# aleph-zero-foundation/sha2-on-cq-halo2

Measured on AMD Instinct MI355X. Metric: sha256_cq_create_proof_k18: MSM Mscalar/s over proof-generation wall-clock (ms_per_step), higher is better.
Workload: dtype u256-montgomery

## Files before the change

### sha2_on_cq_halo2_amd/csrc/capi_msm.hip

```cpp
#include <algorithm>
#include <cstdlib>
#include <cstring>
#include <string>
#include <vector>
#include "ctx.hpp"
#include "msm.hpp"
#include "g1fft.hpp"
#include "setup.hpp"
#include "cq.hpp"
#include "serde.hpp"
#include "msm_g2.hpp"

using namespace cq;

uint32_t msm_table_window_bits(size_t n) {
  if (const char* e = getenv("CQ_TABLE_C")) {
    const long v = atol(e);
    if (v >= (long)MSM_TABLE_C_MIN && v <= (long)MSM_TABLE_C_MAX) return (uint32_t)v;
  }
  return n >= ((size_t)1 << 20) ? 17u : MSM_TABLE_C;
}

static uint32_t pick_c(cq_ctx* c, uint32_t n) {
  if (c->msm_c) return c->msm_c;
// ... 243 lines not shown
  c->msm_precompute = on != 0;
  return CQ_OK;
}

int cq_msm_set_table_window(cq_ctx* c, uint32_t bits) {
  if (!c || (bits != 0 && (bits < MSM_TABLE_C_MIN || bits > MSM_TABLE_C_MAX))) return CQ_ERR_ARG;
  c->msm_table_c = bits;
  return CQ_OK;
}

int cq_msm_table_width_dev(cq_ctx* c, const uint64_t* bases_dev, size_t n, uint32_t preferred_bits, uint32_t* bits) {
  if (!c || !bases_dev || !bits) return CQ_ERR_ARG;
  const cq_ctx::MsmTable* t = c->find_msm_table(bases_dev, n, nullptr, preferred_bits);
  *bits = t ? t->c : 0;
  return CQ_OK;
}

int cq_msm_bucket_sums_dev(cq_ctx* c, const uint64_t* const* bases_dev, size_t arrays, int packed, const uint32_t* index_dev, size_t n,
                           size_t buckets, uint64_t* out_dev) {
  if (!c || !bases_dev || !index_dev || !out_dev || !arrays || arrays > MSM_MAX_BATCH || !n || n > ((size_t)1 << 26) || !buckets ||
      buckets > ((size_t)1 << (MSM_TABLE_C - 1)))
    return CQ_ERR_ARG;
  CQ_HIP(c, hipSetDevice(c->device));
  void *sc, *conv = nullptr;
  int rc;
  if ((rc = c->ensure_scratch(Scratch::EntryA, n * sizeof(Fr), &sc)) != CQ_OK) return rc;
  if (!packed && (rc = c->ensure_scratch(Scratch::EntryB, arrays * n * sizeof(G1Affine), &conv)) != CQ_OK) return rc;
  if (msm_index_scalars(c, index_dev, (uint32_t)n, (uint32_t)buckets, (Fr*)sc) != 0) return c->fail(CQ_ERR_HIP, "bucket sums: scalars");
  std::vector<const Fr*> scal(arrays, (const Fr*)sc);
  std::vector<const G1Affine*> bs(arrays);
  for (size_t a = 0; a < arrays; a++) {
    if (!bases_dev[a]) return CQ_ERR_ARG;
    bs[a] = (const G1Affine*)bases_dev[a];
    if (!packed) {
      G1Affine* dst = (G1Affine*)conv + a * n;
      if (msm_bases29(c, bs[a], (uint32_t)n, dst) != 0) return c->fail(CQ_ERR_HIP, "bucket sums: bases");
      bs[a] = dst;
    }
  }
  if (msm_bucket_sums(c, scal.data(), bs.data(), (uint32_t)n, (uint32_t)arrays, (uint32_t)buckets, (G1Affine*)out_dev) != 0)
    return c->fail(CQ_ERR_HIP, "bucket-sum launch failed");
  return c->wait(c->stream);
}

int cq_msm_set_window(cq_ctx* c, uint32_t bits) {
  if (!c || (bits != 0 && (bits < 2 || bits > 15))) return CQ_ERR_ARG;
  c->msm_c = bits;
  return CQ_OK;
}

int cq_best_multiexp_dev(cq_ctx* c, const uint64_t* coeffs_dev, const uint64_t* bases_dev, size_t len,
                         uint64_t out_jac[12]) {
  if (!c || !out_jac || (len && (!coeffs_dev || !bases_dev))) return CQ_ERR_ARG;
  CQ_HIP(c, hipSetDevice(c->device));
  const Fr* sc = (const Fr*)coeffs_dev;
  return msm_batch(c, &sc, (const G1Affine*)bases_dev, len, 1, out_jac);
}

int cq_msm_batch_dev(cq_ctx* c, const uint64_t* const* coeffs_dev, const uint64_t* bases_dev, size_t len,
                     size_t count, uint64_t* out_jac) {
  if (!c || !out_jac || !coeffs_dev || (len && !bases_dev)) return CQ_ERR_ARG;
  CQ_HIP(c, hipSetDevice(c->device));
  return msm_batch(c, (const Fr* const*)coeffs_dev, (const G1Affine*)bases_dev, len, count, out_jac);
// ... 414 lines not shown
```

### sha2_on_cq_halo2_amd/csrc/cq.hip

```cpp
#include "cq.hpp"
#include "ctx.hpp"
#include "tablehash.hpp"

namespace cq {

__global__ void table_insert_kernel(const Fr* __restrict__ values, uint32_t N, uint32_t* __restrict__ slots, uint32_t nslots,
                                    uint32_t* __restrict__ err) {
  const uint32_t i = blockIdx.x * blockDim.x + threadIdx.x;
  if (i >= N) return;
  const Fr v = ld(values + i);
  uint32_t s = hash_fr(v) & (nslots - 1);
  for (uint32_t probe = 0; probe < nslots; probe++) {
    const uint32_t prev = atomicCAS(&slots[s], EMPTY, i);
    if (prev == EMPTY) return;
    if (prev != i && ld(values + prev) == v) {
      atomicExch(err, 1u);
      return;
    }
    s = (s + 1) & (nslots - 1);
  }
  atomicExch(err, 2u);
}

constexpr uint32_t R1_ROWS = 4;
__global__ __launch_bounds__(256) void cq_round1_kernel(CqRound1Batch batch, uint32_t u, uint32_t* __restrict__ err) {
  const CqRound1Args& a = batch.a[blockIdx.y];
  uint32_t* __restrict__ m_counts = batch.m_counts[blockIdx.y];
  Fr* __restrict__ bucket = batch.bucket[blockIdx.y];
  uint32_t found[R1_ROWS];
#pragma unroll
  for (uint32_t r = 0; r < R1_ROWS; r++) {
    const uint32_t row = (blockIdx.x * R1_ROWS + r) * blockDim.x + threadIdx.x;
    uint32_t idx = EMPTY;
    bool bad = row >= u;
    for (uint32_t j = 0; !bad && j < a.width; j++) {
      const Fr v = ld(a.cols[j] + row);
      const uint32_t ix = table_find(a.values[j], a.slots[j], a.nslots[j], v);
      if (ix == EMPTY) {
        atomicExch(err, 1u);
        bad = true;
      } else if (j && ix != idx) {
        atomicExch(err, 2u);
        bad = true;
      }
      idx = ix;
    }
    found[r] = bad ? EMPTY : idx;
    if (bucket && row < batch.n) st(bucket + row, row >= u ? Fr::from_u64(batch.blind_bucket + 1) : bad ? Fr::zero() : Fr::from_u64(idx + 1));
  }
  uint32_t held = EMPTY, held_cnt = 0;
#pragma unroll
  for (uint32_t r = 0; r < R1_ROWS; r++) {
    if (found[r] == EMPTY) continue;
    if (found[r] == held) {
      held_cnt++;
    } else {
      if (held_cnt) atomicAdd(&m_counts[held], held_cnt);
      held = found[r];
      held_cnt = 1;
    }
  }
  bool pending = held_cnt != 0;
#pragma unroll 1
  for (int round = 0; round < 4 && __ballot(pending); round++) {
    const unsigned long long pend = __ballot(pending);
    const int leader = __ffsll((long long)pend) - 1;
    const uint32_t lidx = __shfl(held, leader, 64);
    const bool mine = pending && held == lidx;
    uint32_t c = mine ? held_cnt : 0u;
#pragma unroll
    for (int d = 32; d >= 1; d >>= 1) c += __shfl_xor(c, d, 64);
// ... 304 lines not shown
```

### sha2_on_cq_halo2_amd/csrc/cq.hpp

```cpp
#pragma once
#include <hip/hip_runtime.h>
#include <vector>
#include "../../include/cq_halo2.h"
#include "curve.hpp"
#include "poly.hpp"

struct cq_ctx;
struct cq_params;

namespace cq {

constexpr uint32_t CQ_MAX_WIDTH = 8;

struct CqRound1Args {
  const Fr* cols[CQ_MAX_WIDTH];
  const Fr* values[CQ_MAX_WIDTH];
  const uint32_t* slots[CQ_MAX_WIDTH];
  uint32_t nslots[CQ_MAX_WIDTH];
  uint32_t width;
};
constexpr uint32_t CQ_ROUND1_BATCH = 8;
struct CqRound1Batch {
  CqRound1Args a[CQ_ROUND1_BATCH];
  uint32_t* m_counts[CQ_ROUND1_BATCH];
  Fr* bucket[CQ_ROUND1_BATCH] = {};
  uint32_t blind_bucket = 0, n = 0;
  uint32_t count;
};
struct CqThetaPowers {
  Fr pow[CQ_MAX_WIDTH];
  uint32_t width;
};
constexpr uint32_t CQ_FOLD_BATCH = 8;
struct CqFoldBatch {
  const Fr* src[CQ_FOLD_BATCH][CQ_MAX_WIDTH];
  uint32_t width[CQ_FOLD_BATCH];
  Fr* out[CQ_FOLD_BATCH];
  const Fr* f[CQ_FOLD_BATCH];
  Fr* b[CQ_FOLD_BATCH];
  const uint32_t* m[CQ_FOLD_BATCH];
  Fr* den[CQ_FOLD_BATCH];
  Fr theta_pow[CQ_MAX_WIDTH];
  uint32_t count;
};
int cq_fold_inputs(cq_ctx* c, const CqFoldBatch& b, uint32_t n);
int cq_round2_prep(cq_ctx* c, const CqFoldBatch& b, uint32_t n, uint32_t N, uint32_t u, const Fr& beta);
struct CqAValuesBatch {
  const Fr* den_inv[CQ_FOLD_BATCH];
// ... 141 lines not shown
```

### sha2_on_cq_halo2_amd/csrc/msm.hip

```cpp
#include <algorithm>
#include <cstdlib>
#include "msm.hpp"
#include "curve29.hpp"
#include "ctx.hpp"

namespace cq {

__global__ __launch_bounds__(256) void msm_set_ptrs_kernel(MsmPtrs sc, MsmPtrs bs, MsmStrides st, MsmStrides ln, MsmStrides src, const void** dst,
                                                          uint32_t batch, uint4* __restrict__ zero, size_t zero_quads) {
  CQ_CRITICAL_WAVES();
  for (size_t i = (size_t)blockIdx.x * blockDim.x + threadIdx.x; i < zero_quads; i += (size_t)gridDim.x * blockDim.x)
    zero[i] = make_uint4(0, 0, 0, 0);
  if (blockIdx.x) return;
  const uint32_t t = threadIdx.x;
  if (t < batch) {
    dst[t] = sc.p[t];
    dst[batch + t] = bs.p[t];
    ((uint64_t*)(dst + 2 * batch))[t] = st.s[t];
    ((uint64_t*)(dst + 3 * batch))[t] = ln.s[t];
    ((uint64_t*)(dst + 4 * batch))[t] = src.s[t];
  }
}

static __device__ __forceinline__ uint32_t signed_digit(const U256& v, uint32_t w, uint32_t c, uint32_t& carry, uint32_t& neg) {
// ... 358 lines not shown
__global__ __launch_bounds__(PART_THREADS) void msm_bucket_place_kernel(const uint32_t* __restrict__ part_pay, const uint8_t* __restrict__ part_low,
                                                                        const uint32_t* __restrict__ poff,
                                                                        const uint32_t* __restrict__ off0, uint32_t* __restrict__ cursor,
                                                                        uint32_t* __restrict__ sorted) {
  CQ_CRITICAL_WAVES();
  part_tile_place(BucketBins<PB>{sorted}, part_pay, part_low, poff, off0, cursor);
}
__global__ __launch_bounds__(PART_THREADS) void msm_refine_count_kernel(const uint16_t* __restrict__ low1, const uint32_t* __restrict__ poff1,
                                                                        uint32_t bins_log, uint32_t* __restrict__ psize2) {
  part_count(RefineBins(bins_log), low1, poff1, psize2);
}
__global__ __launch_bounds__(PART_THREADS) void msm_refine_place_kernel(const uint32_t* __restrict__ pay1, const uint16_t* __restrict__ low1,
                                                                        const uint32_t* __restrict__ poff1, uint32_t bins_log,
                                                                        const uint32_t* __restrict__ poff2, uint32_t* __restrict__ cursor2,
                                                                        uint32_t* __restrict__ pay2, uint8_t* __restrict__ low2) {
  part_tile_place(RefineBins(bins_log, pay2, low2), pay1, low1, poff1, poff2, cursor2);
}

__global__ __launch_bounds__(256) void msm_alias_counts_kernel(uint32_t* __restrict__ counts, const uint64_t* __restrict__ list_src, uint32_t B) {
  CQ_CRITICAL_WAVES();
  const uint32_t m = blockIdx.y, src = (uint32_t)list_src[m];
  const uint32_t i = blockIdx.x * blockDim.x + threadIdx.x;
  if (src != m && i < B) counts[(size_t)m * B + i] = counts[(size_t)src * B + i];
}

static __device__ __forceinline__ uint32_t level_value(uint32_t cnt, uint32_t lv, uint32_t s1) {
  if (lv == 0) return cnt;
  uint32_t t = (cnt + s1 - 1) / s1;
  for (uint32_t k = 2; k <= lv; k++) t = t <= MSM_SHORT_MIN ? 0 : (t + MSM_S2 - 1) / MSM_S2;
  return t;
}
static __device__ __forceinline__ uint32_t combine_short_limit(uint32_t slots) {
  return slots <= MSM_WAVE_BUDGET ? MSM_SHORT_MIN : MSM_SHORT;
}

static __device__ __forceinline__ uint32_t block_excl_scan256(uint32_t v, uint32_t* sh , uint32_t& total) {
  const uint32_t lane = threadIdx.x & 63, wid = threadIdx.x >> 6;
  uint32_t x = v;
#pragma unroll
  for (int off = 1; off < 64; off <<= 1) {
    uint32_t y = __shfl_up(x, off, 64);
    if ((int)lane >= off) x += y;
  }
  __syncthreads();
  if (lane == 63) sh[wid] = x;
  __syncthreads();
// ... 240 lines not shown
    r.x = a.x * (iv * a.zzz);
    r.y = a.y * (iv * a.zz);
  }
  store_affine29(next + i, {Fq29::from_mont256(r.x), Fq29::from_mont256(r.y)});
}

int msm_precompute_tables(cq_ctx* ctx, const G1Affine* bases, uint32_t n, uint32_t c, G1Affine* table ) {
  const uint32_t W = (255 + c - 1) / c;
  hipStream_t s = ctx->stream;
  msm_table0_kernel<<<(n + 255) / 256, 256, 0, s>>>(bases, table, n);
  for (uint32_t w = 1; w < W; w++)
    msm_pre_kernel<<<(n + 255) / 256, 256, 0, s>>>(table + (size_t)(w - 1) * n, table + (size_t)w * n, n, c);
  return hipGetLastError() == hipSuccess ? 0 : -1;
}

__global__ __launch_bounds__(256) void msm_bases29_kernel(const G1Affine* bases, G1Affine* out, uint32_t n) {
  const uint32_t i = blockIdx.x * blockDim.x + threadIdx.x;
  if (i >= n) return;
  const Affine29 p = load_affine29(bases + i, true);
  store_affine29(out + i, p);
}
int msm_bases29(cq_ctx* ctx, const G1Affine* bases, uint32_t n, G1Affine* out) {
  msm_bases29_kernel<<<(n + 255) / 256, 256, 0, ctx->stream>>>(bases, out, n);
  return hipGetLastError() == hipSuccess ? 0 : -1;
}
__global__ __launch_bounds__(256) void msm_index_scalars_kernel(const uint32_t* __restrict__ index, uint32_t n, uint32_t count, Fr* __restrict__ out) {
  const uint32_t i = blockIdx.x * blockDim.x + threadIdx.x;
  if (i >= n) return;
  const uint32_t j = index[i];
  out[i] = j < count ? Fr::from_u64(j + 1) : Fr::zero();
}
int msm_index_scalars(cq_ctx* ctx, const uint32_t* index, uint32_t n, uint32_t count, Fr* out) {
  msm_index_scalars_kernel<<<(n + 255) / 256, 256, 0, ctx->stream>>>(index, n, count, out);
  return hipGetLastError() == hipSuccess ? 0 : -1;
}

__global__ __launch_bounds__(256) void msm_buckets_affine_kernel(const XYZZ* __restrict__ buckets, const uint32_t* __restrict__ t1, uint32_t B,
                                                                 uint32_t count, G1Affine* __restrict__ out) {
  const uint32_t i = blockIdx.x * blockDim.x + threadIdx.x, m = blockIdx.y;
  if (i >= count) return;
  const size_t g = (size_t)m * B + i;
  G1Affine r = G1Affine::identity();
  if (t1[g]) {
    const XYZZ29 v = load_xyzz29(buckets + g);
    if (!v.is_identity()) {
      const Fq x = v.x.reduced().to_mont256(), y = v.y.to_mont256(), zz = v.zz.to_mont256(), zzz = v.zzz.to_mont256();
      const Fq iv = (zz * zzz).inv();
      r.x = x * (iv * zzz);
      r.y = y * (iv * zz);
    }
  }
  G1Affine* o = out + (size_t)m * count + i;
  uint32_t w[8];
  for (int k = 0; k < 8; k++) w[k] = r.x.v.l[k];
  st8(&o->x, w);
  for (int k = 0; k < 8; k++) w[k] = r.y.v.l[k];
// ... 354 lines not shown
  off_pairs = o;   o = up(o + (size_t)batch * Wb * (rows + cols) * sizeof(XYZZ));
  total = o;
}

struct PartPass1 {
  hipStream_t s;
  dim3 hgrid, sgrid;
  const Fr* const* scalars;
  const uint64_t *lens, *list_src;
  uint32_t c, W, npart, per_lane, batch, s1, P;
  uint32_t *psize , *poff, *s1_dev, *part_pay;
  void* part_low;
};
template <uint32_t CW, uint32_t NW, typename LowT>
static void launch_part_pass1(const PartPass1& a) {
  msm_part_hist_kernel<CW, NW><<<a.hgrid, DIGITS_LDS_THREADS, 0, a.s>>>(a.scalars, a.lens, a.c, a.W, a.npart, a.per_lane, a.psize);
  msm_part_scan_kernel<<<1, 1024, 0, a.s>>>(a.psize, a.P, a.poff, a.list_src, a.batch, a.npart, a.s1, a.s1_dev);
  msm_part_scatter_kernel<CW, NW, LowT><<<a.sgrid, PSC_THREADS, 0, a.s>>>(a.scalars, a.lens, a.c, a.W, a.npart, a.poff, a.psize + a.P, a.part_pay,
                                                                          (LowT*)a.part_low);
}

int msm_run(cq_ctx* ctx, const Fr* const* scalars_host_ptrs, const G1Affine* const* bases_host_ptrs, const size_t* lens,
            uint32_t n, uint32_t c, uint32_t batch, bool pre, const size_t* table_strides, void* workspace,
            G1Jac* window_sums_dev, G1Affine* raw_out, uint32_t raw_count) {
  hipStream_t s = ctx->stream;
  MsmLayout L(n, c, batch, pre);
  if (pre && (n > (1u << 26) || L.W > 32)) return -4;
  if (L.tmax[0] > 0xfffffff0ull || (uint64_t)batch * L.W * n > 0xfffffff0ull) return -3;
  char* ws = (char*)workspace;
  const Fr** d_scalars = (const Fr**)(ws + L.off_ptrs);
  const G1Affine** d_bases = (const G1Affine**)(ws + L.off_ptrs) + batch;
  uint32_t* ranks = (uint32_t*)(ws + L.off_ranks);
  uint32_t* counts = (uint32_t*)(ws + L.off_counts);
  XYZZ* buckets = (XYZZ*)(ws + L.off_buckets);
  uint32_t* blocksums = (uint32_t*)(ws + L.off_blocksums);
  uint32_t* ticket = (uint32_t*)(ws + L.off_ticket);
  uint32_t* s1_dev = blocksums + (size_t)L.nseq * L.nblk;
  uint32_t* off = (uint32_t*)(ws + L.off_off);
  uint32_t* tk = (uint32_t*)(ws + L.off_tk);
  uint32_t* sorted = (uint32_t*)(ws + L.off_sorted);
  XYZZ* part[2] = {(XYZZ*)(ws + L.off_part[0]), (XYZZ*)(ws + L.off_part[1])};
  XYZZ* pairs = (XYZZ*)(ws + L.off_pairs);
  const uint32_t M = L.M, W = L.W, Bt = L.Bt;
  if (batch == 0 || batch > MSM_MAX_BATCH) return -2;
  MsmPtrs sp, bp;
  MsmStrides stv, lnv, srcv;
  uint32_t alias[MSM_MAX_BATCH];
  bool any_alias = false;
  for (uint32_t i = 0; i < MSM_MAX_BATCH; i++) {
    sp.p[i] = i < batch ? (const void*)scalars_host_ptrs[i] : nullptr;
    bp.p[i] = i < batch ? (const void*)bases_host_ptrs[i] : nullptr;
    stv.s[i] = (i < batch && pre) ? (uint64_t)table_strides[i] : 0;
    lnv.s[i] = i < batch ? (uint64_t)lens[i] : 0;
    alias[i] = i;
    if (i < batch && L.part_sort)
      for (uint32_t j = 0; j < i; j++)
        if (alias[j] == j && scalars_host_ptrs[j] == scalars_host_ptrs[i] && lens[j] == lens[i] && lens[i]) {
          alias[i] = j;
          lnv.s[i] = 0;
          any_alias = true;
          break;
        }
    srcv.s[i] = alias[i];
  }
  const uint64_t* d_strides = (const uint64_t*)((const void**)d_scalars + 2 * batch);
  const uint64_t* d_lens = (const uint64_t*)((const void**)d_scalars + 3 * batch);
  const uint64_t* d_src = (const uint64_t*)((const void**)d_scalars + 4 * batch);
  uint64_t load = 0;
  for (uint32_t i = 0; i < batch; i++) load = std::max<uint64_t>(load, (uint64_t)lens[i] * W / (L.Wb * M));
  const uint32_t partials = pre && L.Wb > 1 ? MSM_PARTIALS_TARGET / 4 : MSM_PARTIALS_TARGET;
  const uint32_t s1 = load <= MSM_S1_BIG_LOAD ? msm_small_launch_s1((uint64_t)batch * W * n)
                                              : std::max<uint32_t>(MSM_S1_BIG, (uint32_t)((load + partials - 1) / partials));
  const uint32_t* off0 = off;
  auto front = [&]() -> int {
  {
    const size_t quads = (L.zero_end - L.off_counts) / sizeof(uint4);
    const uint32_t blocks = (uint32_t)std::min<size_t>((quads + 255) / 256, 1024);
    msm_set_ptrs_kernel<<<std::max(blocks, 1u), 256, 0, s>>>(sp, bp, stv, lnv, srcv, (const void**)d_scalars, batch, (uint4*)counts, quads);
  }
  if (L.part_sort) {
    const uint32_t P = batch * L.npart;
    const uint64_t E = (uint64_t)batch * W * n;
    uint32_t* part_pay = (uint32_t*)(ws + L.off_ranks);
    void* part_low = part_pay + (L.mid ? 2 * E : E);
    uint32_t* poff = (uint32_t*)(ws + L.off_poff);
    uint32_t* cursor = (uint32_t*)(ws + L.off_cursor);
    uint32_t* psize = (uint32_t*)(ws + L.off_psize);
    const uint32_t per_lane = (uint64_t)n * batch <= (1u << 21) ? 2u : DIGITS_LDS_PER_LANE;
    const uint32_t hist_chunk = DIGITS_LDS_THREADS * per_lane;
    const dim3 hgrid((n + hist_chunk - 1) / hist_chunk, batch), sgrid((n + PSC_THREADS - 1) / PSC_THREADS, batch);
    const PartPass1 pp{s, hgrid, sgrid, d_scalars, d_lens, d_src, c, W, L.npart, per_lane, batch, s1, P, psize, poff, s1_dev, part_pay, part_low};
    if (c == 15 && W == 17) launch_part_pass1<15, 17, uint8_t>(pp);
    else if (c == 16 && W == 16) launch_part_pass1<16, 16, uint8_t>(pp);
    else if (c == 17 && W == 15) launch_part_pass1<17, 15, uint8_t>(pp);
    else if (c == 18 && W == 15) launch_part_pass1<18, 15, uint16_t>(pp);
    else if (c == 19 && W == 14) launch_part_pass1<19, 14, uint16_t>(pp);
    else if (c == 20 && W == 13) launch_part_pass1<20, 13, uint16_t>(pp);
    else if (L.mid) launch_part_pass1<0, 0, uint16_t>(pp);
    else launch_part_pass1<0, 0, uint8_t>(pp);
    auto split_for = [&](uint32_t parts) {
      const uint64_t tiles = (uint64_t)W * n * batch / ((uint64_t)parts * PART_TILE) + 1;
      return (uint32_t)std::min<uint64_t>(PART_SPLIT, tiles);
    };
// ... 13 lines not shown
      msm_part_scan_kernel<<<1, 1024, 0, s>>>(psize2, F, poff2);
      msm_refine_place_kernel<<<dim3(P, PART_SPLIT), PART_THREADS, 0, s>>>(part_pay, low1, poff, bins_log, poff2, psize2 + F, pay2, low2);
      fpay = pay2;
      flow = low2;
      fpoff = poff2;
    }
    const uint32_t split = split_for(F);
    const bool wide = !L.mid && L.shift1 == PART_BITS_WIDE;
    if (wide) msm_bucket_count_kernel<PART_BITS_WIDE><<<dim3(F, split), PART_THREADS, 0, s>>>(flow, fpoff, counts);
    else msm_bucket_count_kernel<PART_BITS><<<dim3(F, split), PART_THREADS, 0, s>>>(flow, fpoff, counts);
    if (any_alias) msm_alias_counts_kernel<<<dim3((L.B + 255) / 256, batch), 256, 0, s>>>(counts, d_src, L.B);
    msm_scan_reduce_kernel<<<L.nblk, 256, 0, s>>>(counts, Bt, L.nseq, s1, s1_dev, blocksums, ticket);
    msm_scan_apply_kernel<<<L.nblk, 256, 0, s>>>(counts, Bt, L.nseq, s1, s1_dev, blocksums, off, tk);
    if (wide) msm_bucket_place_kernel<PART_BITS_WIDE><<<dim3(F, split), PART_THREADS, 0, s>>>(fpay, flow, fpoff, off0, cursor, sorted);
    else msm_bucket_place_kernel<PART_BITS><<<dim3(F, split), PART_THREADS, 0, s>>>(fpay, flow, fpoff, off0, cursor, sorted);
  } else {
    msm_digits_kernel<<<dim3((n + 255) / 256, batch), 256, 0, s>>>(d_scalars, d_lens, n, c, W, pre ? 1u : 0u, ranks, counts);
    msm_scan_reduce_kernel<<<L.nblk, 256, 0, s>>>(counts, Bt, L.nseq, s1, nullptr, blocksums, ticket);
    msm_scan_apply_kernel<<<L.nblk, 256, 0, s>>>(counts, Bt, L.nseq, s1, nullptr, blocksums, off, tk);
    msm_scatter_kernel<<<dim3((n + 255) / 256, batch), 256, 0, s>>>(d_scalars, d_lens, n, c, W, pre ? 1u : 0u, ranks, off0, sorted);
  }
  return 0;
  };
  std::vector<uint64_t> sig{(uint64_t)(uintptr_t)workspace, (uint64_t)(uintptr_t)window_sums_dev, n, c, batch, pre ? 1u : 0u, s1,
                            (uint64_t)(uintptr_t)raw_out, raw_count};
  for (uint32_t i = 0; i < batch; i++) {
    sig.push_back((uint64_t)(uintptr_t)scalars_host_ptrs[i]);
    sig.push_back((uint64_t)(uintptr_t)bases_host_ptrs[i]);
    sig.push_back((uint64_t)lens[i]);
    sig.push_back(pre ? (uint64_t)table_strides[i] : 0);
  }
  if (ctx->run_graph(sig, 0, front) != 0) return -1;
  if (ctx->prof_on && ctx->prof_entries && ctx->prof_entries_n < cq_ctx::PROF_COUNTERS)
    (void)hipMemcpyAsync(ctx->prof_entries + ctx->prof_entries_n++, off0 + Bt, sizeof(uint32_t), hipMemcpyDeviceToHost, s);
  constexpr size_t TAIL_EARLY_POINTS = (size_t)1 << 20;
  const bool tail_early = n >= TAIL_EARLY_POINTS;
  if (tail_early && ctx->msm_tail_event) {
    (void)hipEventRecord(ctx->msm_tail_event, s);
    ctx->msm_tail_seq++;
  }
  hipEvent_t pe = ctx->prof_begin(CQ_PROF_MSM_ACCUMULATE);
  msm_accumulate_kernel<<<(uint32_t)((L.tmax[0] + MSM_ACC_THREADS - 1) / MSM_ACC_THREADS), MSM_ACC_THREADS, 0, s>>>(
      d_bases, L.B, pre ? 1u : 0u, d_strides, d_src, sorted, counts, off0, tk, off + (size_t)(Bt + 1), Bt, part[0], buckets);
  ctx->prof_end(pe);
  if (ctx->msm_tail_event && !tail_early) {
    (void)hipEventRecord(ctx->msm_tail_event, s);
    ctx->msm_tail_seq++;
  }
  auto tail = [&]() -> int {
  for (uint32_t k = 1; k < L.levels; k++) {
// ... 19 lines not shown
  const uint32_t sets = batch * L.Wb;
  constexpr uint32_t QUAD_ROWCOL_SETS = 4, SEG32_SETS = 12;
  if (sets <= QUAD_ROWCOL_SETS)
    msm_rowcol_quad_kernel<<<dim3(L.rows + L.cols, sets), 256, 0, s>>>(buckets, tk, M, L.rows, L.cols, pairs);
  else if (sets <= SEG32_SETS)
    msm_rowcol_kernel<32><<<dim3((L.rows + L.cols + 1) / 2, sets), 64, 0, s>>>(buckets, tk, M, L.rows, L.cols, pairs);
  else
    msm_rowcol_kernel<16><<<dim3((L.rows + L.cols + 3) / 4, sets), 64, 0, s>>>(buckets, tk, M, L.rows, L.cols, pairs);
  constexpr uint32_t QUAD_WEIGHTED_WAVES = 2048;
  if (sets * MSM_SET_POINTS * 4 <= QUAD_WEIGHTED_WAVES) msm_weighted_quad_kernel<<<MSM_SET_POINTS * sets, 256, 0, s>>>(pairs, L.rows, L.cols, window_sums_dev);
  else msm_weighted_kernel<<<MSM_SET_POINTS * sets, 64, 0, s>>>(pairs, L.rows, L.cols, window_sums_dev);
  return 0;
  };
  if (ctx->run_graph(sig, 1, tail) != 0) return -1;
  return hipGetLastError() == hipSuccess ? 0 : -1;
}

bool msm_bucket_sums_fit(uint32_t n, uint32_t batch) {
  if (!batch || batch > MSM_MAX_BATCH || !n || n > (1u << 26)) return false;
  MsmLayout L(n, MSM_TABLE_C, batch, true);
  return (uint64_t)batch * L.W * n <= 0xfffffff0ull && L.tmax[0] <= 0xfffffff0ull && L.total <= ((size_t)32 << 30);
}

int msm_bucket_sums(cq_ctx* ctx, const Fr* const* scalars, const G1Affine* const* bases29, uint32_t n, uint32_t batch, uint32_t count,
                    G1Affine* out) {
  const uint32_t c = MSM_TABLE_C;
  if (!count || count > (1u << (c - 1)) || !msm_bucket_sums_fit(n, batch)) return -2;
  MsmLayout L(n, c, batch, true);
  void* ws;
  if (ctx->ensure_scratch(Scratch::MsmWork, L.total, &ws) != 0) return -1;
  const std::vector<size_t> lens(batch, n), strides(batch, n);
  return msm_run(ctx, scalars, bases29, lens.data(), n, c, batch, true, strides.data(), ws, nullptr, out, count);
}

G1Jac msm_set_value(const G1Jac* planes, uint32_t cols) {
  G1Jac v = planes[6];
  for (int t = 5; t >= 0; t--) v = jac_add(jac_dbl(v), planes[t]);
  if (cols == 128) {
    for (int t = 6; t >= 0; t--) v = jac_add(jac_dbl(v), planes[7 + t]);
    return jac_add(v, planes[14]);
  }
  G1Jac u = planes[13];
  for (int t = 5; t >= 0; t--) u = jac_add(jac_dbl(u), planes[7 + t]);
  for (uint32_t l = cols; l > 1; l >>= 1) v = jac_dbl(v);
  return jac_add(jac_add(v, u), planes[14]);
}

G1Jac msm_fold_sets(const G1Jac* pairs, uint32_t Wb, uint32_t M, uint32_t cols) {
  if (Wb == 1) return msm_set_value(pairs, cols);
  G1Jac planes[MSM_SET_POINTS];
  for (uint32_t q = 0; q < MSM_SET_POINTS; q++) {
    planes[q] = pairs[q];
    for (uint32_t s = 1; s < Wb; s++) planes[q] = jac_add(planes[q], pairs[(size_t)MSM_SET_POINTS * s + q]);
  }
  G1Jac acc = msm_set_value(planes, cols);
// ... 29 lines not shown
```

### sha2_on_cq_halo2_amd/csrc/msm.hpp

```cpp
#pragma once
#include <hip/hip_runtime.h>
#include <vector>
#include "curve.hpp"

struct cq_ctx;

namespace cq {

constexpr uint32_t MSM_ACC_THREADS = 128;

#ifndef CQ_MSM_S1
#define CQ_MSM_S1 24
#endif
constexpr uint32_t MSM_S1 = CQ_MSM_S1;
#ifndef CQ_MSM_S1_BIG
#define CQ_MSM_S1_BIG 32
#endif
#ifndef CQ_MSM_S1_BIG_LOAD
#define CQ_MSM_S1_BIG_LOAD 512
#endif
constexpr uint32_t MSM_S1_BIG = CQ_MSM_S1_BIG;
constexpr uint32_t MSM_S1_BIG_LOAD = CQ_MSM_S1_BIG_LOAD;
#ifndef CQ_MSM_PARTIALS_TARGET
#define CQ_MSM_PARTIALS_TARGET 48
// ... 29 lines not shown
#endif
constexpr uint32_t MSM_SHORT_MAX = CQ_MSM_SHORT_MAX;
static_assert(MSM_SHORT_MAX <= MSM_SHORT_LIMIT && MSM_SHORT_MAX >= 4097, "the cut-over covers N + 1 = 4097 and fits the kernel");

struct MsmPtrs {
  const void* p[MSM_MAX_BATCH];
};
struct MsmStrides {
  uint64_t s[MSM_MAX_BATCH];
};

struct MsmLayout {
  uint32_t n, c, batch, W, Wb, M, B, Bt, levels, nseq, nblk, rows, cols, npart, nfinal, shift1;
  bool pre, part_sort, mid;
  uint64_t tmax[8];
  size_t off_ptrs, off_ranks, off_poff, off_poff2, off_counts, off_cursor, off_psize, off_psize2, off_buckets, off_ticket, zero_end, off_blocksums,
      off_off, off_tk, off_sorted, off_part[2], off_pairs, total;
  MsmLayout(uint32_t n_, uint32_t c_, uint32_t batch_, bool pre_ = false);
};

uint32_t msm_window_bits(uint32_t n);
int msm_run(cq_ctx* ctx, const Fr* const* scalars, const G1Affine* const* bases, const size_t* lens, uint32_t n, uint32_t c,
            uint32_t batch, bool pre, const size_t* table_strides, void* workspace, G1Jac* window_sums_dev,
            G1Affine* raw_out = nullptr, uint32_t raw_count = 0);
size_t msm_short_workspace(uint32_t n, uint32_t batch);
int msm_short_run(cq_ctx* ctx, const Fr* const* scalars, const G1Affine* const* bases, uint32_t n, uint32_t batch, void* workspace,
                  G1Jac* window_sums_dev);
int msm_bucket_sums(cq_ctx* ctx, const Fr* const* scalars, const G1Affine* const* bases29, uint32_t n, uint32_t batch, uint32_t count,
                    G1Affine* out);
int msm_bases29(cq_ctx* ctx, const G1Affine* bases, uint32_t n, G1Affine* out);
int msm_index_scalars(cq_ctx* ctx, const uint32_t* index, uint32_t n, uint32_t count, Fr* out);
bool msm_bucket_sums_fit(uint32_t n, uint32_t batch);
int msm_precompute_tables(cq_ctx* ctx, const G1Affine* bases, uint32_t n, uint32_t c, G1Affine* table);
G1Jac msm_set_value(const G1Jac* planes, uint32_t cols);
G1Jac msm_fold_windows(const G1Jac* pairs, uint32_t W, uint32_t c, uint32_t cols);
G1Jac msm_fold_sets(const G1Jac* pairs, uint32_t Wb, uint32_t M, uint32_t cols);

}

int cq_msm_multi(cq_ctx* c, const cq::Fr* const* scalars, const cq::G1Affine* const* bases, size_t len, size_t count,
                 uint64_t* out_jac);
int cq_msm_multi_v(cq_ctx* c, const cq::Fr* const* scalars, const cq::G1Affine* const* bases, const size_t* lens, size_t count,
                   uint64_t* out_jac);
struct MsmPending {
  struct Launch {
    size_t first = 0, slot = 0;
    uint32_t batch = 0, c = 0, nmax = 0, W = 0, Wb = 0, M = 0, cols = 0;
    bool pre = false, empty = false;
    bool short_path = false;
  };
  std::vector<Launch> launches;
  void* host = nullptr;
  size_t slots = 0, count = 0;
};
// ... 10 lines not shown
```

### sha2_on_cq_halo2_amd/csrc/prover.hip

```cpp
#include <algorithm>
#include <array>
#include <atomic>
#include <chrono>
#include <cstdio>
#include <cstdlib>
#include <cstring>
#include <thread>
#include <vector>
#include "blake2b.hpp"
#include "comm.hpp"
#include "cq.hpp"
#include "ctx.hpp"
#include "msm.hpp"
#include "plonk.hpp"
#include "prover.hpp"
#include "glv.hpp"
#include "xoshiro.hpp"

using namespace cq;

namespace {

struct Transcript {
  Blake2b st;
// ... 561 lines not shown
        ga.prog = pk->lookup_prog + lk.prog[j];
        ga.num_polys = 1;
        ga.constants = pk->constants;
        ga.challenges = B.challenges;
        ga.advice = B.adv;
        ga.fixed = pk->fixed_values;
        ga.instance = B.inst_lag;
        ga.stride = n;
        ga.size = (uint32_t)n;
        ga.rot_scale = 1;
        ga.y = Fr::zero();
        Fr* dst = B.lk_inputs + input_slot * n;
        CQ_TRY(gate_eval(c, ga, dst));
        lk_input[l][j] = dst;
      }
      CqRound1Args& ra = r1b.a[r1b.count];
      ra.width = w;
      for (uint32_t j = 0; j < w; j++) {
        ra.cols[j] = lk_input[l][j];
        ra.values[j] = lk.tables[j]->values;
        ra.slots[j] = lk.tables[j]->slots;
        ra.nslots[j] = lk.tables[j]->nslots;
      }
      r1b.bucket[r1b.count] = b_by_rows ? bpoly + l * n : nullptr;
      r1b.n = b_by_rows ? (uint32_t)n : 0;
      r1b.blind_bucket = (uint32_t)N;
      r1b.m_counts[r1b.count++] = m_counts_ + l * N;
      if (r1b.count == CQ_ROUND1_BATCH || l + 1 == L) {
        CQ_TRY(cq_round1(c, r1b, u, err_dev_));
        r1b.count = 0;
      }
    }
    CQ_TRY(cq_m_to_fr(c, m_counts_, (uint32_t)(L * N), B.m_fr));
    for (size_t l0 = 0; b_by_rows && l0 < L; l0 += MSM_MAX_BATCH / 2) {
      std::vector<const Fr*> sc;
      std::vector<const G1Affine*> bs;
      for (size_t l = l0; l < std::min(L, l0 + MSM_MAX_BATCH / 2); l++)
        for (int q = 0; q < 2; q++) { sc.push_back(bpoly + l * n); bs.push_back(pk->b_row_bases[q]); }
      if (msm_bucket_sums(c, sc.data(), bs.data(), (uint32_t)n, (uint32_t)sc.size(), (uint32_t)(N + 1), B.b_sums + 2 * l0 * (N + 1)) != 0)
        return c->fail(CQ_ERR_HIP, "bucket-sum launch failed");
    }
    *herr = 0;
    CQ_HIP(c, hipMemcpyAsync((void*)herr, err_dev_, 4, hipMemcpyDeviceToHost, s));
    return CQ_OK;
  };
  auto lookup_error = [&]() -> int {
    if (*herr == 1) return c->fail(CQ_ERR_LOOKUP, "witness value not in table");
    if (*herr == 2) return c->fail(CQ_ERR_LOOKUP, "Vector lookup must be on the same table row");
    return CQ_OK;
  };
  const bool early_m = L > 0 && pk->num_phases == 1 && pk->challenge_phase.empty();
  std::vector<G1Affine> m_commitments(L, G1Affine::identity());

  const size_t NC = pk->challenge_phase.size();
  std::vector<Fr> user_challenges(NC, Fr::zero());
  std::vector<G1Affine> advice_commitments(A, G1Affine::identity());
  auto phase_of = [&](size_t a) -> uint32_t { return pk->advice_phase.empty() ? 0u : pk->advice_phase[a]; };
  for (uint32_t phase = 0; phase < pk->num_phases; phase++) {
    const bool last_phase = phase + 1 == pk->num_phases;
    std::vector<size_t> cols;
    for (size_t a = 0; a < A; a++)
// ... 945 lines not shown
```

Baseline: 1186.

## Feed bucket-sum MSM with raw row indices instead of Fr scalars

```diff
diff --git a/sha2_on_cq_halo2_amd/csrc/capi_msm.hip b/sha2_on_cq_halo2_amd/csrc/capi_msm.hip
--- a/sha2_on_cq_halo2_amd/csrc/capi_msm.hip
+++ b/sha2_on_cq_halo2_amd/csrc/capi_msm.hip
@@ -289,12 +289,10 @@
       buckets > ((size_t)1 << (MSM_TABLE_C - 1)))
     return CQ_ERR_ARG;
   CQ_HIP(c, hipSetDevice(c->device));
-  void *sc, *conv = nullptr;
+  void* conv = nullptr;
   int rc;
-  if ((rc = c->ensure_scratch(Scratch::EntryA, n * sizeof(Fr), &sc)) != CQ_OK) return rc;
   if (!packed && (rc = c->ensure_scratch(Scratch::EntryB, arrays * n * sizeof(G1Affine), &conv)) != CQ_OK) return rc;
-  if (msm_index_scalars(c, index_dev, (uint32_t)n, (uint32_t)buckets, (Fr*)sc) != 0) return c->fail(CQ_ERR_HIP, "bucket sums: scalars");
-  std::vector<const Fr*> scal(arrays, (const Fr*)sc);
+  std::vector<const uint32_t*> idx(arrays, index_dev);
   std::vector<const G1Affine*> bs(arrays);
   for (size_t a = 0; a < arrays; a++) {
     if (!bases_dev[a]) return CQ_ERR_ARG;
@@ -305,7 +303,7 @@
       bs[a] = dst;
     }
   }
-  if (msm_bucket_sums(c, scal.data(), bs.data(), (uint32_t)n, (uint32_t)arrays, (uint32_t)buckets, (G1Affine*)out_dev) != 0)
+  if (msm_bucket_sums(c, idx.data(), bs.data(), (uint32_t)n, (uint32_t)arrays, (uint32_t)buckets, (G1Affine*)out_dev) != 0)
     return c->fail(CQ_ERR_HIP, "bucket-sum launch failed");
   return c->wait(c->stream);
 }
diff --git a/sha2_on_cq_halo2_amd/csrc/cq.hip b/sha2_on_cq_halo2_amd/csrc/cq.hip
--- a/sha2_on_cq_halo2_amd/csrc/cq.hip
+++ b/sha2_on_cq_halo2_amd/csrc/cq.hip
@@ -26,7 +26,7 @@
 __global__ __launch_bounds__(256) void cq_round1_kernel(CqRound1Batch batch, uint32_t u, uint32_t* __restrict__ err) {
   const CqRound1Args& a = batch.a[blockIdx.y];
   uint32_t* __restrict__ m_counts = batch.m_counts[blockIdx.y];
-  Fr* __restrict__ bucket = batch.bucket[blockIdx.y];
+  uint32_t* __restrict__ bucket = batch.bucket[blockIdx.y];
   uint32_t found[R1_ROWS];
 #pragma unroll
   for (uint32_t r = 0; r < R1_ROWS; r++) {
@@ -46,7 +46,7 @@
       idx = ix;
     }
     found[r] = bad ? EMPTY : idx;
-    if (bucket && row < batch.n) st(bucket + row, row >= u ? Fr::from_u64(batch.blind_bucket + 1) : bad ? Fr::zero() : Fr::from_u64(idx + 1));
+    if (bucket && row < batch.n) bucket[row] = row >= u ? batch.blind_bucket : bad ? EMPTY : idx;
   }
   uint32_t held = EMPTY, held_cnt = 0;
 #pragma unroll
diff --git a/sha2_on_cq_halo2_amd/csrc/cq.hpp b/sha2_on_cq_halo2_amd/csrc/cq.hpp
--- a/sha2_on_cq_halo2_amd/csrc/cq.hpp
+++ b/sha2_on_cq_halo2_amd/csrc/cq.hpp
@@ -23,7 +23,7 @@
 struct CqRound1Batch {
   CqRound1Args a[CQ_ROUND1_BATCH];
   uint32_t* m_counts[CQ_ROUND1_BATCH];
-  Fr* bucket[CQ_ROUND1_BATCH] = {};
+  uint32_t* bucket[CQ_ROUND1_BATCH] = {};
   uint32_t blind_bucket = 0, n = 0;
   uint32_t count;
 };
diff --git a/sha2_on_cq_halo2_amd/csrc/msm.hip b/sha2_on_cq_halo2_amd/csrc/msm.hip
--- a/sha2_on_cq_halo2_amd/csrc/msm.hip
+++ b/sha2_on_cq_halo2_amd/csrc/msm.hip
@@ -404,6 +404,163 @@
   const uint32_t m = blockIdx.y, src = (uint32_t)list_src[m];
   const uint32_t i = blockIdx.x * blockDim.x + threadIdx.x;
   if (src != m && i < B) counts[(size_t)m * B + i] = counts[(size_t)src * B + i];
+}
+
+constexpr uint32_t INDEX_THREADS = 256, INDEX_PER_LANE = 8, INDEX_TILE = INDEX_THREADS * INDEX_PER_LANE;
+constexpr uint32_t INDEX_SLOTS = 2 * INDEX_TILE, INDEX_NONE = 0xffffffffu;
+constexpr uint32_t INDEX_RANK_BITS = 12;
+static_assert(INDEX_TILE <= (1u << INDEX_RANK_BITS) && INDEX_SLOTS <= (1u << (31 - INDEX_RANK_BITS)), "slot and rank share a word");
+
+static __device__ __forceinline__ uint32_t index_slot(uint32_t* keys, uint32_t b) {
+  uint32_t s = (b * 0x9e3779b1u) >> 20 & (INDEX_SLOTS - 1);
+  for (uint32_t probe = 0; probe < INDEX_SLOTS; probe++) {
+    const uint32_t prev = atomicCAS(&keys[s], INDEX_NONE, b);
+    if (prev == INDEX_NONE || prev == b) break;
+    s = (s + 1) & (INDEX_SLOTS - 1);
+  }
+  return s;
+}
+
+__global__ __launch_bounds__(INDEX_THREADS) void msm_index_count_kernel(const uint32_t* const* __restrict__ index, const uint64_t* __restrict__ lens,
+                                                                        const uint64_t* __restrict__ list_src, uint32_t batch, uint32_t B,
+                                                                        uint32_t count, uint32_t* __restrict__ counts, uint32_t* totals ,
+                                                                        uint32_t* ticket, uint32_t s1_host, uint32_t* __restrict__ s1_out) {
+  CQ_CRITICAL_WAVES();
+  __shared__ uint32_t keys[INDEX_SLOTS], cnt[INDEX_SLOTS];
+  __shared__ uint32_t tile_total;
+  const uint32_t m = blockIdx.y, t = threadIdx.x, lane = t & 63;
+  const uint32_t len = (uint32_t)lens[m];
+  const uint32_t base = blockIdx.x * INDEX_TILE;
+  if (base < len) {
+    for (uint32_t s = t; s < INDEX_SLOTS; s += INDEX_THREADS) {
+      keys[s] = INDEX_NONE;
+      cnt[s] = 0;
+    }
+    if (t == 0) tile_total = 0;
+    __syncthreads();
+    const uint32_t* __restrict__ idx = index[m];
+    uint32_t bk[INDEX_PER_LANE];
+#pragma unroll
+    for (uint32_t k = 0; k < INDEX_PER_LANE; k++) {
+      const uint32_t i = base + k * INDEX_THREADS + t;
+      bk[k] = i < len ? idx[i] : INDEX_NONE;
+    }
+    uint32_t held = INDEX_NONE, held_cnt = 0;
+#pragma unroll
+    for (uint32_t k = 0; k < INDEX_PER_LANE; k++) {
+      if (bk[k] >= count) continue;
+      if (bk[k] == held) {
+        held_cnt++;
+      } else {
+        if (held_cnt) atomicAdd(&cnt[index_slot(keys, held)], held_cnt);
+        held = bk[k];
+        held_cnt = 1;
+      }
+    }
+    bool pending = held_cnt != 0;
+#pragma unroll 1
+    for (int round = 0; round < 2 && __ballot(pending); round++) {
+      const int leader = __ffsll((long long)__ballot(pending)) - 1;
+      const uint32_t lb = __shfl(held, leader, 64);
+      const bool mine = pending && held == lb;
+      uint32_t c = mine ? held_cnt : 0u;
+#pragma unroll
+      for (int d = 32; d >= 1; d >>= 1) c += __shfl_xor(c, d, 64);
+      if ((int)lane == leader) atomicAdd(&cnt[index_slot(keys, lb)], c);
+      if (mine) pending = false;
+    }
+    if (pending) atomicAdd(&cnt[index_slot(keys, held)], held_cnt);
+    __syncthreads();
+    uint32_t sum = 0;
+    for (uint32_t s = t; s < INDEX_SLOTS; s += INDEX_THREADS) {
+      const uint32_t h = cnt[s];
+      if (h) atomicAdd(&counts[(size_t)m * B + keys[s]], h);
+      sum += h;
+    }
+#pragma unroll
+    for (int d = 32; d >= 1; d >>= 1) sum += __shfl_xor(sum, d, 64);
+    if (lane == 0 && sum) atomicAdd(&tile_total, sum);
+    __syncthreads();
+    if (t == 0 && tile_total) atomicAdd(&totals[m], tile_total);
+  }
+  if (t) return;
+  __threadfence();
+  if (atomicAdd(ticket, 1u) != gridDim.x * gridDim.y - 1) return;
+  __threadfence();
+  uint64_t entries = 0;
+  for (uint32_t q = 0; q < batch; q++) entries += atomicAdd(&totals[(uint32_t)list_src[q]], 0u);
+  const uint32_t s1 = msm_small_launch_s1(entries);
+  *s1_out = entries < (uint64_t)MSM_S1 * MSM_SMALL_LANES && s1 < s1_host ? s1 : s1_host;
+}
+
+__global__ __launch_bounds__(INDEX_THREADS) void msm_index_place_kernel(const uint32_t* const* __restrict__ index, const uint64_t* __restrict__ lens,
+                                                                        uint32_t B, uint32_t count, const uint32_t* __restrict__ off0,
+                                                                        uint32_t* __restrict__ cursor, uint32_t* __restrict__ sorted) {
+  CQ_CRITICAL_WAVES();
+  __shared__ uint32_t keys[INDEX_SLOTS], run[INDEX_SLOTS];
+  const uint32_t m = blockIdx.y, t = threadIdx.x, lane = t & 63;
+  const uint32_t len = (uint32_t)lens[m];
+  const uint32_t base = blockIdx.x * INDEX_TILE;
+  if (base >= len) return;
+  for (uint32_t s = t; s < INDEX_SLOTS; s += INDEX_THREADS) {
+    keys[s] = INDEX_NONE;
+    run[s] = 0;
+  }
+  __syncthreads();
+  const uint32_t* __restrict__ idx = index[m];
+  uint32_t bk[INDEX_PER_LANE], where[INDEX_PER_LANE];
+#pragma unroll
+  for (uint32_t k = 0; k < INDEX_PER_LANE; k++) {
+    const uint32_t i = base + k * INDEX_THREADS + t;
+    bk[k] = i < len ? idx[i] : INDEX_NONE;
+  }
+#pragma unroll
+  for (uint32_t k = 0; k < INDEX_PER_LANE; k++) {
+    const bool act = bk[k] < count;
+    bool pending = act, issue = act;
+    uint32_t add = 1, lead = 64, below = 0;
+#pragma unroll
+    for (int round = 0; round < 2; round++) {
+      const unsigned long long pend = __ballot(pending);
+      if (pend) {
+        const int leader = __ffsll((long long)pend) - 1;
+        const uint32_t lb = __shfl(bk[k], leader, 64);
+        const bool mine = pending && bk[k] == lb;
+        const unsigned long long grp = __ballot(mine);
+        if (mine) {
+          lead = (uint32_t)leader;
+          below = __popcll(grp & ((1ull << lane) - 1ull));
+          add = __popcll(grp);
+          issue = (int)lane == leader;
+          pending = false;
+        }
+      }
+    }
+    uint32_t slot = 0, first = 0;
+    if (issue) {
+      slot = index_slot(keys, bk[k]);
+      first = atomicAdd(&run[slot], add);
+    }
+    const uint32_t lslot = __shfl(slot, lead & 63, 64), lfirst = __shfl(first, lead & 63, 64);
+    if (lead < 64) {
+      slot = lslot;
+      first = lfirst + below;
+    }
+    where[k] = act ? (slot << INDEX_RANK_BITS) | first : INDEX_NONE;
+  }
+  __syncthreads();
+  for (uint32_t s = t; s < INDEX_SLOTS; s += INDEX_THREADS) {
+    const uint32_t h = run[s];
+    if (h) {
+      const size_t g = (size_t)m * B + keys[s];
+      run[s] = off0[g] + atomicAdd(&cursor[g], h);
+    }
+  }
+  __syncthreads();
+#pragma unroll
+  for (uint32_t k = 0; k < INDEX_PER_LANE; k++)
+    if (where[k] != INDEX_NONE)
+      sorted[run[where[k] >> INDEX_RANK_BITS] + (where[k] & ((1u << INDEX_RANK_BITS) - 1u))] = base + k * INDEX_THREADS + t;
 }
 
 static __device__ __forceinline__ uint32_t level_value(uint32_t cnt, uint32_t lv, uint32_t s1) {
@@ -690,16 +847,6 @@
 }
 int msm_bases29(cq_ctx* ctx, const G1Affine* bases, uint32_t n, G1Affine* out) {
   msm_bases29_kernel<<<(n + 255) / 256, 256, 0, ctx->stream>>>(bases, out, n);
-  return hipGetLastError() == hipSuccess ? 0 : -1;
-}
-__global__ __launch_bounds__(256) void msm_index_scalars_kernel(const uint32_t* __restrict__ index, uint32_t n, uint32_t count, Fr* __restrict__ out) {
-  const uint32_t i = blockIdx.x * blockDim.x + threadIdx.x;
-  if (i >= n) return;
-  const uint32_t j = index[i];
-  out[i] = j < count ? Fr::from_u64(j + 1) : Fr::zero();
-}
-int msm_index_scalars(cq_ctx* ctx, const uint32_t* index, uint32_t n, uint32_t count, Fr* out) {
-  msm_index_scalars_kernel<<<(n + 255) / 256, 256, 0, ctx->stream>>>(index, n, count, out);
   return hipGetLastError() == hipSuccess ? 0 : -1;
 }
 
@@ -1100,9 +1247,12 @@
 
 int msm_run(cq_ctx* ctx, const Fr* const* scalars_host_ptrs, const G1Affine* const* bases_host_ptrs, const size_t* lens,
             uint32_t n, uint32_t c, uint32_t batch, bool pre, const size_t* table_strides, void* workspace,
-            G1Jac* window_sums_dev, G1Affine* raw_out, uint32_t raw_count) {
+            G1Jac* window_sums_dev, G1Affine* raw_out, uint32_t raw_count, const uint32_t* const* index_host_ptrs) {
   hipStream_t s = ctx->stream;
   MsmLayout L(n, c, batch, pre);
+  const bool by_index = index_host_ptrs != nullptr;
+  if (by_index && (!L.part_sort || L.Wb != 1 || !raw_out || raw_count > L.B)) return -2;
+  auto list_ptr = [&](uint32_t i) -> const void* { return by_index ? (const void*)index_host_ptrs[i] : (const void*)scalars_host_ptrs[i]; };
   if (pre && (n > (1u << 26) || L.W > 32)) return -4;
   if (L.tmax[0] > 0xfffffff0ull || (uint64_t)batch * L.W * n > 0xfffffff0ull) return -3;
   char* ws = (char*)workspace;
@@ -1126,14 +1276,14 @@
   uint32_t alias[MSM_MAX_BATCH];
   bool any_alias = false;
   for (uint32_t i = 0; i < MSM_MAX_BATCH; i++) {
-    sp.p[i] = i < batch ? (const void*)scalars_host_ptrs[i] : nullptr;
+    sp.p[i] = i < batch ? list_ptr(i) : nullptr;
     bp.p[i] = i < batch ? (const void*)bases_host_ptrs[i] : nullptr;
     stv.s[i] = (i < batch && pre) ? (uint64_t)table_strides[i] : 0;
     lnv.s[i] = i < batch ? (uint64_t)lens[i] : 0;
     alias[i] = i;
     if (i < batch && L.part_sort)
       for (uint32_t j = 0; j < i; j++)
-        if (alias[j] == j && scalars_host_ptrs[j] == scalars_host_ptrs[i] && lens[j] == lens[i] && lens[i]) {
+        if (alias[j] == j && list_ptr(j) == list_ptr(i) && lens[j] == lens[i] && lens[i]) {
           alias[i] = j;
           lnv.s[i] = 0;
           any_alias = true;
@@ -1156,7 +1306,17 @@
     const uint32_t blocks = (uint32_t)std::min<size_t>((quads + 255) / 256, 1024);
     msm_set_ptrs_kernel<<<std::max(blocks, 1u), 256, 0, s>>>(sp, bp, stv, lnv, srcv, (const void**)d_scalars, batch, (uint4*)counts, quads);
   }
-  if (L.part_sort) {
+  if (by_index) {
+    uint32_t* cursor = (uint32_t*)(ws + L.off_cursor);
+    uint32_t* totals = (uint32_t*)(ws + L.off_psize);
+    const dim3 grid((n + INDEX_TILE - 1) / INDEX_TILE, batch);
+    const uint32_t* const* d_index = (const uint32_t* const*)d_scalars;
+    msm_index_count_kernel<<<grid, INDEX_THREADS, 0, s>>>(d_index, d_lens, d_src, batch, L.B, raw_count, counts, totals, totals + batch, s1, s1_dev);
+    if (any_alias) msm_alias_counts_kernel<<<dim3((L.B + 255) / 256, batch), 256, 0, s>>>(counts, d_src, L.B);
+    msm_scan_reduce_kernel<<<L.nblk, 256, 0, s>>>(counts, Bt, L.nseq, s1, s1_dev, blocksums, ticket);
+    msm_scan_apply_kernel<<<L.nblk, 256, 0, s>>>(counts, Bt, L.nseq, s1, s1_dev, blocksums, off, tk);
+    msm_index_place_kernel<<<grid, INDEX_THREADS, 0, s>>>(d_index, d_lens, L.B, raw_count, off0, cursor, sorted);
+  } else if (L.part_sort) {
     const uint32_t P = batch * L.npart;
     const uint64_t E = (uint64_t)batch * W * n;
     uint32_t* part_pay = (uint32_t*)(ws + L.off_ranks);
@@ -1216,10 +1376,10 @@
   }
   return 0;
   };
-  std::vector<uint64_t> sig{(uint64_t)(uintptr_t)workspace, (uint64_t)(uintptr_t)window_sums_dev, n, c, batch, pre ? 1u : 0u, s1,
+  std::vector<uint64_t> sig{(uint64_t)(uintptr_t)workspace, (uint64_t)(uintptr_t)window_sums_dev, n, c, batch, (pre ? 1u : 0u) | (by_index ? 2u : 0u), s1,
                             (uint64_t)(uintptr_t)raw_out, raw_count};
   for (uint32_t i = 0; i < batch; i++) {
-    sig.push_back((uint64_t)(uintptr_t)scalars_host_ptrs[i]);
+    sig.push_back((uint64_t)(uintptr_t)list_ptr(i));
     sig.push_back((uint64_t)(uintptr_t)bases_host_ptrs[i]);
     sig.push_back((uint64_t)lens[i]);
     sig.push_back(pre ? (uint64_t)table_strides[i] : 0);
@@ -1285,7 +1445,7 @@
   return (uint64_t)batch * L.W * n <= 0xfffffff0ull && L.tmax[0] <= 0xfffffff0ull && L.total <= ((size_t)32 << 30);
 }
 
-int msm_bucket_sums(cq_ctx* ctx, const Fr* const* scalars, const G1Affine* const* bases29, uint32_t n, uint32_t batch, uint32_t count,
+int msm_bucket_sums(cq_ctx* ctx, const uint32_t* const* index, const G1Affine* const* bases29, uint32_t n, uint32_t batch, uint32_t count,
                     G1Affine* out) {
   const uint32_t c = MSM_TABLE_C;
   if (!count || count > (1u << (c - 1)) || !msm_bucket_sums_fit(n, batch)) return -2;
@@ -1293,7 +1453,7 @@
   void* ws;
   if (ctx->ensure_scratch(Scratch::MsmWork, L.total, &ws) != 0) return -1;
   const std::vector<size_t> lens(batch, n), strides(batch, n);
-  return msm_run(ctx, scalars, bases29, lens.data(), n, c, batch, true, strides.data(), ws, nullptr, out, count);
+  return msm_run(ctx, nullptr, bases29, lens.data(), n, c, batch, true, strides.data(), ws, nullptr, out, count, index);
 }
 
 G1Jac msm_set_value(const G1Jac* planes, uint32_t cols) {
diff --git a/sha2_on_cq_halo2_amd/csrc/msm.hpp b/sha2_on_cq_halo2_amd/csrc/msm.hpp
--- a/sha2_on_cq_halo2_amd/csrc/msm.hpp
+++ b/sha2_on_cq_halo2_amd/csrc/msm.hpp
@@ -75,14 +75,13 @@
 uint32_t msm_window_bits(uint32_t n);
 int msm_run(cq_ctx* ctx, const Fr* const* scalars, const G1Affine* const* bases, const size_t* lens, uint32_t n, uint32_t c,
             uint32_t batch, bool pre, const size_t* table_strides, void* workspace, G1Jac* window_sums_dev,
-            G1Affine* raw_out = nullptr, uint32_t raw_count = 0);
+            G1Affine* raw_out = nullptr, uint32_t raw_count = 0, const uint32_t* const* index = nullptr);
 size_t msm_short_workspace(uint32_t n, uint32_t batch);
 int msm_short_run(cq_ctx* ctx, const Fr* const* scalars, const G1Affine* const* bases, uint32_t n, uint32_t batch, void* workspace,
                   G1Jac* window_sums_dev);
-int msm_bucket_sums(cq_ctx* ctx, const Fr* const* scalars, const G1Affine* const* bases29, uint32_t n, uint32_t batch, uint32_t count,
+int msm_bucket_sums(cq_ctx* ctx, const uint32_t* const* index, const G1Affine* const* bases29, uint32_t n, uint32_t batch, uint32_t count,
                     G1Affine* out);
 int msm_bases29(cq_ctx* ctx, const G1Affine* bases, uint32_t n, G1Affine* out);
-int msm_index_scalars(cq_ctx* ctx, const uint32_t* index, uint32_t n, uint32_t count, Fr* out);
 bool msm_bucket_sums_fit(uint32_t n, uint32_t batch);
 int msm_precompute_tables(cq_ctx* ctx, const G1Affine* bases, uint32_t n, uint32_t c, G1Affine* table);
 G1Jac msm_set_value(const G1Jac* planes, uint32_t cols);
diff --git a/sha2_on_cq_halo2_amd/csrc/prover.hip b/sha2_on_cq_halo2_amd/csrc/prover.hip
--- a/sha2_on_cq_halo2_amd/csrc/prover.hip
+++ b/sha2_on_cq_halo2_amd/csrc/prover.hip
@@ -607,7 +607,7 @@
         ra.slots[j] = lk.tables[j]->slots;
         ra.nslots[j] = lk.tables[j]->nslots;
       }
-      r1b.bucket[r1b.count] = b_by_rows ? bpoly + l * n : nullptr;
+      r1b.bucket[r1b.count] = b_by_rows ? (uint32_t*)(bpoly + l * n) : nullptr;
       r1b.n = b_by_rows ? (uint32_t)n : 0;
       r1b.blind_bucket = (uint32_t)N;
       r1b.m_counts[r1b.count++] = m_counts_ + l * N;
@@ -618,10 +618,10 @@
     }
     CQ_TRY(cq_m_to_fr(c, m_counts_, (uint32_t)(L * N), B.m_fr));
     for (size_t l0 = 0; b_by_rows && l0 < L; l0 += MSM_MAX_BATCH / 2) {
-      std::vector<const Fr*> sc;
+      std::vector<const uint32_t*> sc;
       std::vector<const G1Affine*> bs;
       for (size_t l = l0; l < std::min(L, l0 + MSM_MAX_BATCH / 2); l++)
-        for (int q = 0; q < 2; q++) { sc.push_back(bpoly + l * n); bs.push_back(pk->b_row_bases[q]); }
+        for (int q = 0; q < 2; q++) { sc.push_back((const uint32_t*)(bpoly + l * n)); bs.push_back(pk->b_row_bases[q]); }
       if (msm_bucket_sums(c, sc.data(), bs.data(), (uint32_t)n, (uint32_t)sc.size(), (uint32_t)(N + 1), B.b_sums + 2 * l0 * (N + 1)) != 0)
         return c->fail(CQ_ERR_HIP, "bucket-sum launch failed");
     }
```

Result: faster. 1299 (median of 6 runs) (+9.5%).
